# antrea-io/theia

Measured on AMD Instinct MI355X. Metric: flow-records/sec, higher is better.
Workload: dtype u64 (aggregates) + f64 (detectors)

## Files before the change

### theia_amd/csrc/tad_capi.cpp

```cpp
#include "tad_engine.h"

using namespace tad;
using namespace tadh;

namespace tadh {

int ensure_rcp_table(JobCtx *e, uint64_t T) {
  const uint64_t want = T + 2;
  if (want <= e->rcp_n) return TAD_OK;
  uint64_t cap = want < 1024 ? 1024 : want + want / 4;
  int rc = ensure(e, e->rcp_table, cap * sizeof(double));
  if (rc != TAD_OK) return rc;
  std::vector<double> h(cap);
  h[0] = 0.0;
  for (uint64_t i = 1; i < cap; ++i) h[i] = 1.0 / (double)i;
  HIP_TRY(e, hipMemcpyAsync(e->rcp_table.p, h.data(), cap * sizeof(double), hipMemcpyHostToDevice, e->stream));
  HIP_TRY(e, hipStreamSynchronize(e->stream));
  e->rcp_n = cap;
  return TAD_OK;
}

int ensure_key_buffers(JobCtx *e, uint64_t K) {
  int rc;
  const uint64_t k = K ? K : 1;
  if ((rc = ensure(e, e->sigma, k * sizeof(double))) != TAD_OK) return rc;
  if ((rc = ensure(e, e->n_pts, k * sizeof(uint32_t))) != TAD_OK) return rc;
  if ((rc = ensure(e, e->n_anom, k * sizeof(uint32_t))) != TAD_OK) return rc;
  if ((rc = ensure(e, e->off, (k + 1) * sizeof(unsigned long long))) != TAD_OK) return rc;
  if ((rc = ensure(e, e->scan_scratch, scan_scratch_elems(k) * sizeof(unsigned long long))) != TAD_OK) return rc;
  if ((rc = ensure(e, e->key_mean, k * sizeof(double))) != TAD_OK) return rc;
  if ((rc = ensure(e, e->key_m2, k * sizeof(double))) != TAD_OK) return rc;
  if ((rc = ensure(e, e->counters, kTailBytes)) != TAD_OK) return rc;
  return TAD_OK;
}

}

namespace {

template <typename Relaunch>
int arima_yield_loop(JobCtx *e, const unsigned int *yielded_dev, Relaunch relaunch) {
  hipStream_t s = e->stream;
  while (yielded_dev != nullptr && e->eng->pause_dev != nullptr) {
    unsigned int y = 0;
    HIP_TRY(e, hipMemcpyAsync(&y, yielded_dev, 4, hipMemcpyDeviceToHost, s));
    HIP_TRY(e, hipStreamSynchronize(s));
    if (y == 0) break;
    const auto t0 = std::chrono::steady_clock::now();
    while (__atomic_load_n(&e->eng->pause_count, __ATOMIC_ACQUIRE) != 0 && std::chrono::steady_clock::now() - t0 < std::chrono::milliseconds(2))
      std::this_thread::sleep_for(std::chrono::microseconds(50));
    const uint32_t grace = __atomic_load_n(&e->eng->pause_count, __ATOMIC_ACQUIRE) != 0 ? 24u : 0u;
    if (relaunch(grace, &yielded_dev) != 0) return fail(e, TAD_ERR_HIP, "ARIMA launch failed");
    e->arima_relaunches++;
  }
  return TAD_OK;
}

int detect_and_count(JobCtx *e, Grid g, JobParams &jp, DevCounters *ctr, uint64_t *rows, bool stats_done = false) {
  hipStream_t s = e->stream;
  int rc;
  if ((rc = ensure_key_buffers(e, g.K)) != TAD_OK) return rc;
  if ((rc = ensure_rcp_table(e, g.T)) != TAD_OK) return rc;
  double *sigma = static_cast<double *>(e->sigma.p);
  uint32_t *n_pts = static_cast<uint32_t *>(e->n_pts.p);
  uint32_t *n_anom = static_cast<uint32_t *>(e->n_anom.p);
  unsigned long long *off = static_cast<unsigned long long *>(e->off.p);

  const bool ewma = jp.algo == TAD_ALGO_EWMA;
  const bool drop = jp.algo == TAD_ALGO_DROP;
  const bool db_fused = jp.algo == TAD_ALGO_DBSCAN && !jp.all_points && !stats_done && dbscan_uses_list(g);
  jp.lazy_sigma = db_fused;
  if (drop) {
    if ((rc = ensure(e, e->calc, (g.K * g.T ? g.K * g.T : 1) * sizeof(double))) != TAD_OK) return rc;
    launch_drop(s, g, jp.drop_nsigma, jp.drop_min_samples, static_cast<double *>(e->calc.p), sigma, n_pts,
                static_cast<double *>(e->key_mean.p), static_cast<double *>(e->key_m2.p), ctr);
  } else if (!stats_done && !db_fused)
    launch_key_sigma(s, g, jp.alpha, ewma && !jp.all_points, static_cast<const double *>(e->rcp_table.p), sigma, n_pts, n_anom, ctr, static_cast<double *>(e->key_mean.p),
                     static_cast<double *>(e->key_m2.p));
  if (jp.algo == TAD_ALGO_DBSCAN) {
    if ((rc = ensure(e, e->aux, dbscan_scratch_bytes(g))) != TAD_OK) return rc;
    if (dbscan_uses_list(g)) {
      DbscanStats dst{nullptr, nullptr, nullptr, nullptr};
      if (db_fused) dst = DbscanStats{n_pts, n_anom, static_cast<double *>(e->key_mean.p), static_cast<double *>(e->key_m2.p)};
      if (launch_dbscan(s, g, jp.eps, jp.min_samples, e->aux.p, dst, jp.settled && db_fused) != 0)
        return fail(e, TAD_ERR_HIP, "DBSCAN launch failed");
    } else {
      return fail(e, TAD_ERR_GRID_TOO_LARGE, "DBSCAN: series of %llu buckets are not supported", (unsigned long long)g.T);
    }
  } else if (jp.algo == TAD_ALGO_ARIMA) {
    if ((rc = ensure(e, e->calc, g.K * g.T * sizeof(double))) != TAD_OK) return rc;
    const size_t wsb = arima_workspace_bytes(g);
    if ((rc = ensure(e, e->aux, wsb)) != TAD_OK) return rc;
    const bool held = e->hold && e->hold->held;
    if (held) e->hold->release();
    const unsigned int *yielded_dev = nullptr;
    if (launch_arima(s, g, sigma, n_pts, jp.maxiter, static_cast<double *>(e->calc.p), ctr, e->aux.p, wsb, e->eng->pause_dev, &yielded_dev) != 0)
      return fail(e, TAD_ERR_HIP, "ARIMA launch failed");
    if ((rc = arima_yield_loop(e, yielded_dev, [&](uint32_t grace, const unsigned int **yd) {
           return launch_arima_fit(s, g, sigma, n_pts, jp.maxiter, static_cast<double *>(e->calc.p), ctr, e->aux.p, e->eng->pause_dev, yd, grace);
         })) != TAD_OK)
      return rc;
    if (held) e->hold->acquire();
  }
  const uint32_t *cnt = n_anom;
  if (jp.all_points && jp.algo != TAD_ALGO_ARIMA && !drop) cnt = n_pts;
  else if (db_fused) {}
  else if (!ewma || jp.all_points) launch_count_flags(s, g, jp.all_points, n_anom);
  launch_scan_moments(s, cnt, off, g.K, static_cast<unsigned long long *>(e->scan_scratch.p), dev_total(e), n_pts,
                      static_cast<const double *>(e->key_mean.p), static_cast<const double *>(e->key_m2.p), dev_moments(e), db_fused ? ctr : nullptr);
  HIP_TRY(e, hipMemcpyAsync(e->tail_host, e->counters.p, kTailBytes, hipMemcpyDeviceToHost, s));
  HIP_TRY(e, hipStreamSynchronize(s));
  HIP_TRY(e, hipGetLastError());
  *rows = *e->total_host;
  return TAD_OK;
}

}

namespace tadh {

void emit_rows(JobCtx *e, Grid g, Lattice L, const JobParams &jp, OutRows out, uint64_t rows) {
  const int kind = jp.algo == TAD_ALGO_EWMA ? 0 : (jp.algo == TAD_ALGO_ARIMA ? 1 : (jp.algo == TAD_ALGO_DROP ? 3 : (jp.lazy_sigma ? 4 : 2)));
  if (kind == 4 && !jp.all_points &&
      launch_emit_dbscan_list(e->stream, g, L, e->aux.p, static_cast<const uint32_t *>(e->n_anom.p), static_cast<const unsigned long long *>(e->off.p), out))
    return;
  launch_emit(e->stream, g, L, kind, jp.all_points, jp.alpha, static_cast<const double *>(e->sigma.p),
              static_cast<const uint32_t *>(e->n_pts.p), static_cast<const double *>(kind == 3 ? e->key_mean.p : e->calc.p),
              static_cast<const unsigned long long *>(e->off.p), out, rows, e->plan.ewma_emit, e->plan.ewma_emit_rows);
}

}

namespace {

int make_result(JobCtx *e, uint64_t rows, bool with_anomaly, tad_mem out_memory, ResultPriv **out, OutRows *dev_rows,
                ResultBlock *dev_block) {
  ResultPriv *rp = new (std::nothrow) ResultPriv();
  if (!rp) return fail(e, TAD_ERR_OUT_OF_MEMORY, "out of host memory");
  memset(rp, 0, sizeof *rp);
  const size_t bytes = result_bytes(rows, with_anomaly);
  int rc = alloc_device_block(e, bytes, dev_block);
  if (rc != TAD_OK) { delete rp; return rc; }
  carve(dev_block->base, rows, with_anomaly, dev_rows);
  rp->pub.n_rows = rows;
  rp->pub.memory = out_memory;
  *out = rp;
  return TAD_OK;
}

int finish_result(JobCtx *e, ResultPriv *rp, uint64_t rows, bool with_anomaly, ResultBlock dev_block, OutRows dev_rows) {
  if (rp->pub.memory == TAD_MEM_DEVICE) {
    rp->block = dev_block.base;
    rp->block_cap = dev_block.cap;
// ... 265 lines not shown
    const FitListArgs fa{wpos, pcnt, loff, list, hb.nv, pcalc, pflag};
    const bool held = e->hold && e->hold->held;
    if (held) e->hold->release();
    const unsigned int *yielded_dev = nullptr;
    if (launch_arima_stream_fit(s, true, nfits, npos, waves, fpos, ysk, sl, fa, jp.maxiter, ctr, e->as_ws.p, e->eng->pause_dev, &yielded_dev, 0) != 0)
      return fail(e, TAD_ERR_HIP, "ARIMA launch failed");
    if ((rc = arima_yield_loop(e, yielded_dev, [&](uint32_t grace, const unsigned int **yd) {
           return launch_arima_stream_fit(s, false, nfits, npos, waves, fpos, ysk, sl, fa, jp.maxiter, ctr, e->as_ws.p, e->eng->pause_dev, yd, grace);
         })) != TAD_OK)
      return rc;
    if (held) e->hold->acquire();
  }
  launch_as_rows(s, P, hb.nk, tidx, sl.ok, pflag, jp.all_points, rows);
  launch_scan(s, rows, row_off, P, scratch, dev_total(e));
  ab->P = P; ab->tidx = tidx; ab->sigma = sl.sigma; ab->pcalc = pcalc; ab->pflag = pflag; ab->rows = rows; ab->row_off = row_off;
  return TAD_OK;
}

int run_sparse_classes(JobCtx *e, const tad_job *job, const JobParams &jp, bool op_max, uint64_t n_rows_in, uint64_t rows_used, uint64_t K, Lattice L,
                       uint64_t P, uint32_t tmax, tad_mem out_memory, tad_result **out);
int sparse_points_direct(JobCtx *e, uint64_t n_rows_in, uint64_t rows_used, Lattice L, uint64_t P, DevCounters *ctr, tad_mem out_memory,
                         tad_points **points_out);

int run_job(tad_engine *eng, const tad_job *job, const tad_columns *cols, tad_mem out_memory, tad_result **out, tad_points **points_out,
            tad_state *stream = nullptr) {
  tad_engine *e = eng;
  const bool points_mode = points_out != nullptr;
  if (stream && e && job && cols) {
    if (job->algo == TAD_ALGO_DBSCAN && !stream->history)
      return fail(e, TAD_ERR_INVALID_ARGUMENT, "tad_run_stream: DBSCAN needs a state with history (tad_state_create_ex with TAD_STATE_HISTORY)");
    if (job->algo == TAD_ALGO_ARIMA && !stream->series)
      return fail(e, TAD_ERR_INVALID_ARGUMENT, "tad_run_stream: ARIMA needs a state with a series (tad_state_create_ex with TAD_STATE_SERIES)");
    if (job->algo != TAD_ALGO_EWMA && job->algo != TAD_ALGO_DBSCAN && job->algo != TAD_ALGO_ARIMA)
      return fail(e, TAD_ERR_INVALID_ARGUMENT, "tad_run_stream: only the EWMA detector has a streaming form, DBSCAN on a state with history and "
                                               "ARIMA on a state with a series (DROP has none)");
    if (cols->num_keys != stream->K) return fail(e, TAD_ERR_INVALID_ARGUMENT, "tad_run_stream: batch declares %llu keys, the state holds %llu (they must be equal)",
                                                 (unsigned long long)cols->num_keys, (unsigned long long)stream->K);
  }
  if (!e) return fail(nullptr, TAD_ERR_INVALID_ARGUMENT, "tad_run: engine is NULL");
  if (!job || !cols || (!out && !points_out)) return fail(e, TAD_ERR_INVALID_ARGUMENT, "tad_run: job, cols and out must not be NULL");
  if (out) *out = nullptr;
  if (points_out) *points_out = nullptr;
  if (!points_mode && job->algo != TAD_ALGO_EWMA && job->algo != TAD_ALGO_ARIMA && job->algo != TAD_ALGO_DBSCAN && job->algo != TAD_ALGO_DROP)
    return fail(e, TAD_ERR_INVALID_ARGUMENT, "invalid request: Throughput Anomaly Detector algorithm type should be 'EWMA' or 'ARIMA' or 'DBSCAN'");
  if (job->agg_flow < TAD_AGG_NONE || job->agg_flow > TAD_AGG_EXTERNAL)
    return fail(e, TAD_ERR_INVALID_ARGUMENT, "invalid request: Throughput Anomaly Detector aggregated flow type should be 'pod' or 'external' or 'svc'");
  if (job->start_time != 0 && job->end_time != 0 && job->end_time <= job->start_time)
    return fail(e, TAD_ERR_INVALID_ARGUMENT, "invalid request: EndInterval should be after StartInterval");
  if (cols->n_rows > 0 && (!cols->key_id || !cols->flow_end_s || !cols->value))
    return fail(e, TAD_ERR_INVALID_ARGUMENT, "tad_run: key_id, flow_end_s and value columns are required");
  if (cols->n_rows > 0 && cols->num_keys == 0)
    return fail(e, TAD_ERR_INVALID_ARGUMENT, "tad_run: num_keys is 0 but there are rows");
  if ((job->flags & TAD_FLAG_KEY_U32) && cols->num_keys >= 0xFFFFFFFFull)
    return fail(e, TAD_ERR_INVALID_ARGUMENT, "tad_run: TAD_FLAG_KEY_U32 needs num_keys < 2^32 - 1 (TAD_KEY_SKIP32 is the skip marker)");
  if (cols->n_buckets > 0 && cols->step < 1)
    return fail(e, TAD_ERR_INVALID_ARGUMENT, "tad_run: lattice hint needs step >= 1");
  if (job->ewma_alpha < 0.0 || job->ewma_alpha > 1.0 || job->dbscan_eps < 0.0 || job->dbscan_min_samples < 0 || job->arima_maxiter < 0 ||
      job->drop_nsigma < 0.0 || job->drop_min_samples < 0)
    return fail(e, TAD_ERR_INVALID_ARGUMENT, "tad_run: detector parameter out of range");

  std::unique_lock<std::mutex> state_lk;
  if (stream) state_lk = std::unique_lock<std::mutex>(stream->mu);
  if (stream && stream->times_stale)
    return fail(e, TAD_ERR_INVALID_ARGUMENT, "tad_run_stream: the series was imported without its times (tad_state_import_times); state unchanged");
  Lease lease(eng, job->id, !points_mode && job->algo == TAD_ALGO_ARIMA);
  if (!lease.c) return fail(eng, TAD_ERR_OUT_OF_MEMORY, "tad_run: no job context available");
  PauseHold hold(eng);
  lease.c->hold = &hold;
  return run_job_locked(lease.c, job, cols, out_memory, out, points_out, stream, 0);
}

int run_job_locked(JobCtx *e, const tad_job *job, const tad_columns *cols, tad_mem out_memory, tad_result **out, tad_points **points_out,
                   tad_state *stream, int depth) {
  const bool points_mode = points_out != nullptr;
  HIP_TRY(e, hipSetDevice(e->device));
  hipStream_t s = e->stream;
  if (depth == 0) {
    e->done.store(0);
    e->total.store(4);
    e->arima_relaunches = 0;
  }

  JobParams jp;
  jp.algo = job->algo;
  jp.alpha = job->ewma_alpha == 0.0 ? 0.5 : job->ewma_alpha;
  jp.eps = job->dbscan_eps == 0.0 ? 250000000.0 : job->dbscan_eps;
  jp.min_samples = job->dbscan_min_samples == 0 ? 4 : job->dbscan_min_samples;
  jp.maxiter = job->arima_maxiter == 0 ? 50 : job->arima_maxiter;
  jp.drop_nsigma = job->drop_nsigma == 0.0 ? 3.0 : job->drop_nsigma;
  jp.drop_min_samples = job->drop_min_samples == 0 ? 3 : job->drop_min_samples;
  jp.all_points = (job->flags & TAD_FLAG_EMIT_ALL_POINTS) != 0;
  const bool op_max = job->value_op == TAD_OP_MAX || (job->value_op == TAD_OP_AUTO && job->agg_flow == TAD_AGG_NONE);
  const uint64_t n = cols->n_rows;
  const uint64_t K = cols->num_keys;
  RowFilter rf{job->start_time, job->end_time};

  int rc;
  const int cw = ((job->flags & TAD_FLAG_KEY_U32) ? kColKey32 : 0) | ((job->flags & TAD_FLAG_TIME_U32) ? kColTime32 : 0);
  const uint64_t kw = (cw & kColKey32) ? 4 : 8, tw = (cw & kColTime32) ? 4 : 8;
  const void *d_key, *d_key2, *d_te, *d_ts, *d_val;
  if ((rc = stage_column(e, e->in_key, cols->key_id, n, cols->memory, &d_key, kw)) != TAD_OK) return rc;
  if ((rc = stage_column(e, e->in_key2, cols->key_id2, n, cols->memory, &d_key2, kw)) != TAD_OK) return rc;
  if ((rc = stage_column(e, e->in_te, cols->flow_end_s, n, cols->memory, &d_te, tw)) != TAD_OK) return rc;
  if ((rc = stage_column(e, e->in_ts, cols->flow_start_s, n, cols->memory, &d_ts, tw)) != TAD_OK) return rc;
  if ((rc = stage_column(e, e->in_val, cols->value, n, cols->memory, &d_val)) != TAD_OK) return rc;

  if ((rc = ensure(e, e->counters, kTailBytes)) != TAD_OK) return rc;
  DevCounters *ctr = static_cast<DevCounters *>(e->counters.p);

  HIP_TRY(e, hipEventRecord(e->ev[0], s));
  if (depth == 0) HIP_TRY(e, hipEventRecord(e->ev[6], s));
  int lat_mode = cols->n_buckets > 0 ? 0 : 1;
  Lattice L = make_lattice(cols->t0, lat_mode == 0 ? cols->step : 1, cols->n_buckets);
  bool empty = (n == 0 || K == 0);
  const tad_plan plan = e->plan;
  const bool force_v1 = plan.stage0 == 1;
  const bool force_v2 = plan.stage0 == 2;
  const bool has2 = cols->key_id2 != nullptr;
  bool force_v1_retry = false;
  bool force_wide_tiles = plan.tile_cells == 1;
  bool force_exact_hist = plan.histogram == 1;
  bool learnt_exact_hist = false, probing_sampled_hist = false;
  bool kh_rejected = false;
  bool sparse_lsd = plan.sparse_sort == 1;
  {
    const JobCtx::Learnt &lt = e->learnt;
    if (depth == 0 && lt.valid && lt.n == n && lt.K == K && lt.has2 == has2 && lt.algo == (int)job->algo && lt.op == (int)op_max) {
      if (lt.exact_hist) {
        if (lt.exact_uses >= lt.exact_backoff) probing_sampled_hist = true;
        else { force_exact_hist = true; learnt_exact_hist = true; }
      }
      if (lt.wide_tiles) force_wide_tiles = true;
    }
  }
  for (int attempt = 0; attempt < 11; ++attempt) {
    const bool hinted = lat_mode == 0;
    HIP_TRY(e, hipMemsetAsync(ctr, 0, kTailMoments, s));
    jp.settled = false;
    bool narrow_tiles = false;
    PartPlan pl{};
    bool v2 = !empty && !force_v1 && !force_v1_retry && (force_v2 || n >= (1ull << 22)) && part_plan_bins(n, K, has2, &pl);
    if (v2 && e->hold) e->hold->acquire();
    if ((rc = ensure(e, e->meta, sizeof(MetaPartial) * kMetaBlocks)) != TAD_OK) return rc;
    int meta_blocks = 0;
    bool hist_sampled = false;
    const tad_key_hist *kh = cols->key_hist;
    bool use_kh = v2 && depth == 0 && !kh_rejected && kh != nullptr && kh->bins != nullptr && lat_mode != 2 && kh->n_rows == n && kh->num_keys == K &&
                  kh->sides == (has2 ? 2u : 1u) && kh->workgroups == (uint32_t)pl.G && kh->nbins == pl.nbins && kh->shift == (uint32_t)pl.shift_bin &&
                  kh->chunk_rows == pl.chunk && rf.end_time == 0 && !(d_ts != nullptr && rf.start_time != 0);
    const uint32_t *binhist = nullptr;
    if (v2) {
      if ((rc = ensure(e, e->binhist, (size_t)pl.G * pl.nbins * 4)) != TAD_OK) return rc;
      hist_sampled = launch_meta_hist(s, (const uint64_t *)d_key, (const uint64_t *)d_key2, (const int64_t *)d_te, (const int64_t *)d_ts, n, K, rf,
                                      pl, static_cast<MetaPartial *>(e->meta.p), static_cast<uint32_t *>(e->binhist.p), ctr, cw,
                                      use_kh ||
                                      (!force_exact_hist && lat_mode != 2 && sampled_slots_bound(n * (has2 ? 2 : 1), pl) < (1ull << 32) &&
                                          (plan.histogram == 2 ||
                                           n * (has2 ? 2 : 1) / ((uint64_t)pl.G * ((K >> kSampleBlockShift) ? (K >> kSampleBlockShift) : 1)) >= 384)));
      meta_blocks = pl.G;
      binhist = static_cast<const uint32_t *>(e->binhist.p);
      if (use_kh && hist_sampled) { binhist = kh->bins; hist_sampled = false; }
      else use_kh = false;
    }
    if (!hinted && !empty && (!v2 || lat_mode == 2)) {
      meta_blocks = (int)((n + 255) / 256);
      if (meta_blocks > kMetaBlocks) meta_blocks = kMetaBlocks;
      launch_meta(s, (const uint64_t *)d_key, (const uint64_t *)d_key2, (const int64_t *)d_te, (const int64_t *)d_ts, n, rf,
                  static_cast<MetaPartial *>(e->meta.p), meta_blocks, cw);
    }
    if (!hinted && !empty) {
      HIP_TRY(e, hipMemcpyAsync(e->meta_host, e->meta.p, sizeof(MetaPartial) * meta_blocks, hipMemcpyDeviceToHost, s));
      HIP_TRY(e, hipStreamSynchronize(s));
      int64_t tmin = 0, tmax = 0, tref = 0;
      uint64_t g = 0, used = 0;
      for (int b = 0; b < meta_blocks; ++b) {
        const MetaPartial &p = e->meta_host[b];
        if (p.used == 0) continue;
        if (used == 0) { tmin = p.tmin; tmax = p.tmax; tref = p.tref; g = p.g; }
        else {
          if (p.tmin < tmin) tmin = p.tmin;
          if (p.tmax > tmax) tmax = p.tmax;
          const uint64_t d = p.tref >= tref ? (uint64_t)p.tref - (uint64_t)tref : (uint64_t)tref - (uint64_t)p.tref;
          g = host_gcd(host_gcd(g, p.g), d);
        }
        used += p.used;
      }
      if (used == 0 && v2 && lat_mode == 1) {
        lat_mode = 2;
        continue;
      }
      if (used == 0) { empty = true; }
      else {
        const uint64_t span = (uint64_t)tmax - (uint64_t)tmin;
        const uint64_t step = host_gcd(host_gcd(g, span), (uint64_t)tref - (uint64_t)tmin);
        L = make_lattice(tmin, (int64_t)(step == 0 ? 1 : step), span / (step == 0 ? 1 : step) + 1);
      }
    }
    HIP_TRY(e, hipEventRecord(e->ev[1], s));
    if (depth == 0) e->done.store(1);
    if (empty) { L = make_lattice(0, 1, 0); v2 = false; }

    uint64_t cells = empty ? 0 : K * L.nb;
    const bool cells_overflow = !empty && L.nb != 0 && cells / L.nb != K;
    uint64_t need = cells * 9 + (jp.algo == TAD_ALGO_ARIMA ? cells * 80 + (1ull << 22) : (jp.algo == TAD_ALGO_DROP ? cells * 8 : 0));
    const uint64_t slots_all = n * (has2 ? 2 : 1);
    bool sparse = !empty && K <= 0xFFFFFFFFull && slots_all < (1ull << 32) &&
                  (plan.sparse == 2 ||
                   (plan.sparse != 1 && (cells_overflow || need > e->ws_limit || (cells >= (1ull << 24) && slots_all < cells / 8))));
    Grid sparse_grid{};
    bool sp_part = false;
    const unsigned long long *stream_poff = nullptr;
    uint64_t stream_P = 0;
    if (sparse && use_kh) {
      kh_rejected = true;
      continue;
    }
    if (sparse) {
      PartPlan spl = pl;
      sp_part = v2 && !sparse_lsd && part_plan_sparse(K, L.nb, has2, &spl);
      if (sp_part) {
        part_plan_wc(slots_all, columns_aligned16(d_key, d_key2, d_te, d_val), has2, 2, &spl);
        if (spl.wc_cap == 0 || slots_all + spl.pad_slots >= (1ull << 32)) sp_part = false;
      }
      if (sp_part && hist_sampled) { force_exact_hist = true; continue; }
      v2 = false;
      const uint64_t stage_slots = slots_all + (sp_part ? spl.pad_slots : 0);
      if ((rc = ensure(e, e->sp_comp_a, stage_slots * 8)) != TAD_OK) return rc;
      if ((rc = ensure(e, e->sp_comp_b, stage_slots * 8)) != TAD_OK) return rc;
      if ((rc = ensure(e, e->sp_val_a, stage_slots * 8)) != TAD_OK) return rc;
      if ((rc = ensure(e, e->sp_val_b, stage_slots * 8)) != TAD_OK) return rc;
      size_t tb = sparse_sort_temp_bytes(slots_all);
      if (sp_part && sparse_part_temp_bytes(spl) > tb) tb = sparse_part_temp_bytes(spl);
      if ((uint64_t)slots_all * 32 + tb > e->ws_limit)
        return fail(e, TAD_ERR_GRID_TOO_LARGE, "sparse Stage 0 needs %llu bytes of sort buffers for %llu row slots > workspace limit %llu",
                    (unsigned long long)(slots_all * 32 + tb), (unsigned long long)slots_all, (unsigned long long)e->ws_limit);
      if ((rc = ensure(e, e->sp_temp, tb + 64)) != TAD_OK) return rc;
      if ((rc = ensure(e, e->sp_first, K * 4 + 64)) != TAD_OK) return rc;
      unsigned long long *d_runs = reinterpret_cast<unsigned long long *>(static_cast<unsigned char *>(e->sp_temp.p) + tb);
      HIP_TRY(e, hipMemsetAsync(d_runs, 0, 16, s));
      HIP_TRY(e, hipEventRecord(e->ev[2], s));
      unsigned long long *ucomp = static_cast<unsigned long long *>(e->sp_comp_a.p), *uval = static_cast<unsigned long long *>(e->sp_val_a.p);
      const uint64_t span = L.nb ? (L.nb - 1) * (uint64_t)L.step : 0;
      if (sp_part) {
        const uint64_t slots = slots_all + spl.pad_slots;
        if ((rc = ensure(e, e->part_total, (size_t)spl.nparts * 4)) != TAD_OK) return rc;
        if ((rc = ensure(e, e->part_start, ((size_t)spl.nparts + 1) * 8)) != TAD_OK) return rc;
        if ((rc = ensure(e, e->part_offs32, (size_t)spl.G * spl.nparts * 4)) != TAD_OK) return rc;
        if ((rc = ensure(e, e->recs, (size_t)slots * 8)) != TAD_OK) return rc;
        if ((rc = ensure(e, e->slices, slice_table_bytes(slots, spl))) != TAD_OK) return rc;
        uint32_t *offs32 = static_cast<uint32_t *>(e->part_offs32.p);
        unsigned long long *part_start = static_cast<unsigned long long *>(e->part_start.p);
        launch_part_offsets(s, binhist, spl, offs32, static_cast<uint32_t *>(e->part_total.p), part_start, false,
                            static_cast<const MetaPartial *>(e->meta.p), n, slots, e->slices.p, Grid{});
        launch_partition(s, (const uint64_t *)d_key, (const uint64_t *)d_key2, (const int64_t *)d_te, (const int64_t *)d_ts, (const uint64_t *)d_val, n, K,
                         rf, L, spl, offs32, part_start, e->recs.p, nullptr, dev_ovf_count(e), 0, ctr, nullptr, nullptr, cw);
        launch_sparse_sort(s, e->recs.p, part_start, binhist, spl, K, L.step, op_max,
                           ucomp, static_cast<unsigned long long *>(e->sp_comp_b.p), static_cast<unsigned long long *>(e->sp_val_b.p),
                           reinterpret_cast<uint32_t *>(uval), e->sp_temp.p, d_runs, ctr);
      } else if (launch_sparse_group(s, (const uint64_t *)d_key, (const uint64_t *)d_key2, (const int64_t *)d_te, (const int64_t *)d_ts, (const uint64_t *)d_val, n, K,
                                     rf, L.t0, span, op_max, ucomp, uval, static_cast<unsigned long long *>(e->sp_comp_b.p),
                                     static_cast<unsigned long long *>(e->sp_val_b.p), e->sp_temp.p, tb, d_runs, ctr, cw) != 0)
        return fail(e, TAD_ERR_HIP, "sparse Stage 0: sort / reduce failed");
      if (depth == 0) e->sp_by_partition = sp_part;
      if (!sp_part) launch_sparse_tmax(s, ucomp, slots_all, d_runs, static_cast<uint32_t *>(e->sp_first.p), reinterpret_cast<unsigned int *>(d_runs + 1));
      unsigned long long runs_tmax[2] = {0, 0};
      HIP_TRY(e, hipMemcpyAsync(runs_tmax, d_runs, 16, hipMemcpyDeviceToHost, s));
      if (sp_part) HIP_TRY(e, hipMemcpyAsync(e->ctr_host, ctr, sizeof(DevCounters), hipMemcpyDeviceToHost, s));
      HIP_TRY(e, hipStreamSynchronize(s));
      if (sp_part) {
        const uint32_t er = e->ctr_host->err;
        if (er & DEV_ERR_KEY_RANGE)
          return fail(e, TAD_ERR_KEY_RANGE, "a key id is >= num_keys (%llu) and is not TAD_KEY_SKIP", (unsigned long long)K);
        if (er & DEV_ERR_OFF_LATTICE) {
          if (lat_mode < 2) { lat_mode = (lat_mode == 0) ? 1 : 2; continue; }
          return fail(e, TAD_ERR_HIP, "internal error: a row fell off the derived time lattice");
        }
        if (er & (DEV_ERR_OVERFLOW_LIST | DEV_ERR_SPARSE_ROUND)) { sparse_lsd = true; continue; }
      }
      const uint64_t P = runs_tmax[0];
      const unsigned int tmax = (unsigned int)runs_tmax[1];
      if (stream) {
        if (sp_part) {
          launch_sparse_compact(s, spl, e->sp_temp.p, static_cast<const unsigned long long *>(e->sp_comp_b.p), static_cast<const unsigned long long *>(e->sp_val_b.p), ucomp, uval);
          launch_sparse_tmax(s, ucomp, slots_all, d_runs, static_cast<uint32_t *>(e->sp_first.p), reinterpret_cast<unsigned int *>(d_runs + 1));
        }
        if ((rc = ensure_key_buffers(e, K)) != TAD_OK) return rc;
        const size_t kpad = (size_t)((K + 3) & ~3ull);
        if ((rc = ensure(e, e->sp_cls, kpad * 4 + (K + 1) * 8 + 64)) != TAD_OK) return rc;
        uint32_t *len = static_cast<uint32_t *>(e->sp_cls.p);
        unsigned long long *poff = reinterpret_cast<unsigned long long *>(len + kpad);
        HIP_TRY(e, hipMemsetAsync(len, 0, (size_t)K * 4, s));
        launch_sparse_len(s, ucomp, P, static_cast<const uint32_t *>(e->sp_first.p), len);
        launch_scan(s, len, poff, K, static_cast<unsigned long long *>(e->scan_scratch.p), nullptr);
        stream_poff = poff;
        stream_P = P;
        sparse_grid = Grid{nullptr, nullptr, K, 0, nullptr};
        HIP_TRY(e, hipEventRecord(e->ev[3], s));
      } else {
        cells = K * (uint64_t)tmax;
        need = cells * 17 + (jp.algo == TAD_ALGO_ARIMA ? cells * 80 + (1ull << 22) : (jp.algo == TAD_ALGO_DROP ? cells * 8 : 0));
        if (P && depth == 0 && (need > e->ws_limit || plan.sparse_classes == 1)) {
          if (sp_part) {
            launch_sparse_compact(s, spl, e->sp_temp.p, static_cast<const unsigned long long *>(e->sp_comp_b.p), static_cast<const unsigned long long *>(e->sp_val_b.p), ucomp, uval);
            launch_sparse_tmax(s, ucomp, slots_all, d_runs, static_cast<uint32_t *>(e->sp_first.p), reinterpret_cast<unsigned int *>(d_runs + 1));
          }
          HIP_TRY(e, hipMemcpyAsync(e->ctr_host, ctr, sizeof(DevCounters), hipMemcpyDeviceToHost, s));
          HIP_TRY(e, hipStreamSynchronize(s));
          const DevCounters c0 = *e->ctr_host;
          if (c0.err & DEV_ERR_KEY_RANGE)
            return fail(e, TAD_ERR_KEY_RANGE, "a key id is >= num_keys (%llu) and is not TAD_KEY_SKIP", (unsigned long long)K);
          if (c0.err & DEV_ERR_OFF_LATTICE) {
            if (lat_mode < 2) { lat_mode = (lat_mode == 0) ? 1 : 2; continue; }
            return fail(e, TAD_ERR_HIP, "internal error: a row fell off the derived time lattice");
          }
          if (points_mode) return sparse_points_direct(e, n, c0.rows_used, L, P, ctr, out_memory, points_out);
          return run_sparse_classes(e, job, jp, op_max, n, c0.rows_used, K, L, P, tmax, out_memory, out);
        }
        if (need > e->ws_limit)
          return fail(e, TAD_ERR_GRID_TOO_LARGE, "sparse point grid needs %llu bytes (%llu keys x longest series %u points) > workspace limit %llu",
                      (unsigned long long)need, (unsigned long long)K, tmax, (unsigned long long)e->ws_limit);
        if ((rc = ensure(e, e->grid_val, (cells ? cells : 1) * 8)) != TAD_OK) return rc;
        if ((rc = ensure(e, e->grid_flag, cells ? cells : 1)) != TAD_OK) return rc;
        if ((rc = ensure(e, e->sp_times, (cells ? cells : 1) * 8)) != TAD_OK) return rc;
        sparse_grid = Grid{static_cast<unsigned long long *>(e->grid_val.p), static_cast<uint8_t *>(e->grid_flag.p), tmax ? K : 0, tmax,
// ... 1034 lines not shown
```

### theia_amd/csrc/tad_stage0_part.hip

```cpp
#include <cstdlib>
#include <cstring>

#include "tad_internal.h"

namespace tad {

static constexpr int kPartThreads = 1024;

static constexpr int kMinCellBits = 15, kMaxCellBits = 24;
static constexpr uint32_t kTileCells = 17744;
static constexpr uint32_t kMaxParts = 2048;
static constexpr size_t kLdsBudget = 156 * 1024;
static constexpr int kGcdSamples = 4;

__device__ __forceinline__ void lds_barrier() { asm volatile("s_waitcnt lgkmcnt(0)\n\ts_barrier" ::: "memory"); }

__device__ __forceinline__ uint64_t p_gcd_u64(uint64_t a, uint64_t b) {
  if (a == 0) return b;
  if (b == 0) return a;
  if (((a | b) >> 32) == 0) {
    uint32_t x = (uint32_t)a, y = (uint32_t)b;
    while (y) { uint32_t r = x % y; x = y; y = r; }
    return x;
  }
  while (b) { uint64_t r = a % b; a = b; b = r; }
  return a;
}

__device__ __forceinline__ uint64_t p_absdiff(int64_t a, int64_t b) {
  return a >= b ? (uint64_t)a - (uint64_t)b : (uint64_t)b - (uint64_t)a;
}

struct PMeta {
  int64_t tmin, tmax, tref;
  uint64_t g, used;
};

__device__ __forceinline__ PMeta pmeta_merge(PMeta a, const PMeta &b) {
  if (b.used == 0) return a;
  if (a.used == 0) return b;
  a.tmin = b.tmin < a.tmin ? b.tmin : a.tmin;
  a.tmax = b.tmax > a.tmax ? b.tmax : a.tmax;
  a.g = p_gcd_u64(p_gcd_u64(a.g, b.g), p_absdiff(a.tref, b.tref));
  a.used += b.used;
  return a;
}

__device__ __forceinline__ bool p_time_kept(int64_t te, int64_t ts, bool has_ts, RowFilter f) {
  if (f.end_time != 0 && !(te < f.end_time)) return false;
  if (f.start_time != 0 && has_ts && !(ts >= f.start_time)) return false;
  return true;
}

__device__ __forceinline__ bool p_bucket(const Lattice &L, int64_t te, uint32_t &bucket) {
  const uint64_t d = (uint64_t)te - (uint64_t)L.t0;
  uint64_t b;
  if (L.mode == 0) b = d;
  else if (L.mode == 1) { if (d >> 32) return false; b = __umul64hi(d, L.magic); }
  else b = d / (uint64_t)L.step;
  if (b >= L.nb || b * (uint64_t)L.step != d) return false;
  bucket = (uint32_t)b;
  return true;
}

struct MetaAcc {
  PMeta m;
  int nsample;
  uint32_t err;
};

#ifndef TAD_WAVE_AGG
#define TAD_WAVE_AGG 1
#endif
#ifndef TAD_ADAPTIVE_QUEUES
#define TAD_ADAPTIVE_QUEUES 1
#endif
#ifndef TAD_WAVE_AGG_MIN
#define TAD_WAVE_AGG_MIN 8
#endif
static constexpr int kWaveAggMin = TAD_WAVE_AGG_MIN;
static constexpr size_t kWcFixedBytes = 18;

__device__ __forceinline__ void hist_add(uint32_t *hist, uint32_t bin, uint32_t weight) {
#if TAD_WAVE_AGG
  const uint32_t b0 = __builtin_amdgcn_readfirstlane(bin);
  const unsigned long long grp = __ballot(bin == b0);
  if (__popcll(grp) >= kWaveAggMin && bin == b0) {
    if (__builtin_amdgcn_mbcnt_hi((uint32_t)(grp >> 32), __builtin_amdgcn_mbcnt_lo((uint32_t)grp, 0u)) == 0) atomicAdd(&hist[b0], (uint32_t)__popcll(grp) * weight);
    return;
  }
#endif
  atomicAdd(&hist[bin], weight);
}

__device__ __forceinline__ void meta_row(MetaAcc &a, uint32_t *hist, uint64_t k1, uint64_t k2, int64_t te, bool kept,
                                         uint64_t K, int shift_bin, uint32_t weight = 1u) {
  if (!kept) return;
  bool counted = false;
  if (k1 != TAD_KEY_SKIP) {
    if (k1 < K) { hist_add(hist, (uint32_t)(k1 >> shift_bin), weight); counted = true; }
    else a.err |= DEV_ERR_KEY_RANGE;
  }
  if (k2 != TAD_KEY_SKIP) {
    if (k2 < K) { hist_add(hist, (uint32_t)(k2 >> shift_bin), weight); counted = true; }
    else a.err |= DEV_ERR_KEY_RANGE;
  }
  if (!counted) return;
  if (a.m.used == 0) {
    a.m.tmin = a.m.tmax = a.m.tref = te;
    a.m.g = 0;
  } else {
    a.m.tmin = te < a.m.tmin ? te : a.m.tmin;
    a.m.tmax = te > a.m.tmax ? te : a.m.tmax;
    if (a.nsample < kGcdSamples) {
      const uint64_t d = p_absdiff(te, a.m.tref);
      if (d != 0) { a.m.g = p_gcd_u64(a.m.g, d); a.nsample++; }
    }
  }
  a.m.used++;
}

__device__ __forceinline__ void hist_row(MetaAcc &a, uint32_t *hist, uint64_t k1, uint64_t k2, uint64_t K, int shift_bin) {
  if (k1 != TAD_KEY_SKIP) {
    if (k1 < K) hist_add(hist, (uint32_t)(k1 >> shift_bin), 1u);
    else a.err |= DEV_ERR_KEY_RANGE;
  }
  if (k2 != TAD_KEY_SKIP) {
    if (k2 < K) hist_add(hist, (uint32_t)(k2 >> shift_bin), 1u);
    else a.err |= DEV_ERR_KEY_RANGE;
  }
}

#ifndef TAD_SAMPLE_MASK
#define TAD_SAMPLE_MASK 15
#endif
#ifndef TAD_REGION_UR
#define TAD_REGION_UR 12
#endif
static constexpr uint32_t kSampleMask = TAD_SAMPLE_MASK;

template <bool VEC, bool HAS2, bool SAMPLE_H, bool K32 = false, bool T32 = false>
__global__ __launch_bounds__(kPartThreads) void k_meta_hist(const uint64_t *__restrict__ key,
                                                            const uint64_t *__restrict__ key2,
                                                            const int64_t *__restrict__ t_end,
                                                            const int64_t *__restrict__ t_start,
                                                            uint64_t n, uint64_t chunk, uint64_t K, RowFilter f,
                                                            int shift_bin, uint32_t nbins,
                                                            MetaPartial *__restrict__ partials,
                                                            uint32_t *__restrict__ binhist, DevCounters *ctr) {
  extern __shared__ __attribute__((aligned(16))) unsigned char smem[];
  uint32_t *hist = reinterpret_cast<uint32_t *>(smem);
  for (uint32_t i = threadIdx.x; i < nbins; i += kPartThreads) hist[i] = 0;
  __syncthreads();
  const uint64_t lo = (uint64_t)blockIdx.x * chunk;
  const uint64_t hi = lo + chunk < n ? lo + chunk : n;
  MetaAcc acc{{0, 0, 0, 0, 0}, 0, 0};
  uint32_t seen = 0;
  const bool has_ts = t_start != nullptr && f.start_time != 0;
  if (VEC) {
    const uint64_t npair = hi > lo ? (hi - lo) >> 1 : 0;
    const ulonglong2 *kv = reinterpret_cast<const ulonglong2 *>(key + lo);
    const ulonglong2 *k2v = reinterpret_cast<const ulonglong2 *>(key2 + (HAS2 ? lo : 0));
    const longlong2 *tv = reinterpret_cast<const longlong2 *>(t_end + lo);
    auto kpair = [&](const ulonglong2 *wide, const uint64_t *col, uint64_t j) -> ulonglong2 {
      if constexpr (K32) return ld_key2<true>(col, lo, j);
      else return wide[j];
    };
    auto tpair = [&](uint64_t j) -> longlong2 {
      if constexpr (T32) return ld_time2<true>(t_end, lo, j);
      else return tv[j];
    };
    constexpr int U = 4;
    const bool sample_t = SAMPLE_H || (f.end_time == 0 && !has_ts);
    uint64_t i = threadIdx.x;
    uint32_t it = 0;
    for (; i + (U - 1) * kPartThreads < npair; i += U * kPartThreads, ++it) {
      const bool zone = (i - threadIdx.x) + 2 * U * kPartThreads >= npair;
      const bool with_t = !sample_t || zone || (it & kSampleMask) == ((threadIdx.x >> 6) & kSampleMask);
      if (SAMPLE_H && !with_t) continue;
      const uint32_t weight = SAMPLE_H && !zone ? kSampleMask + 1u : 1u;
      seen += 2 * U;
      ulonglong2 k[U], k2[U];
      longlong2 t[U];
#pragma unroll
      for (int u = 0; u < U; ++u) {
        k[u] = kpair(kv, key, i + u * kPartThreads);
        k2[u] = HAS2 ? kpair(k2v, key2, i + u * kPartThreads) : make_ulonglong2(TAD_KEY_SKIP, TAD_KEY_SKIP);
      }
      if (with_t) {
#pragma unroll
        for (int u = 0; u < U; ++u) t[u] = tpair(i + u * kPartThreads);
#pragma unroll
        for (int u = 0; u < U; ++u) {
          const uint64_t r = lo + 2 * (i + u * kPartThreads);
          const int64_t ts0 = has_ts ? ld_time<T32>(t_start, r) : 0, ts1 = has_ts ? ld_time<T32>(t_start, r + 1) : 0;
          meta_row(acc, hist, k[u].x, k2[u].x, t[u].x, p_time_kept(t[u].x, ts0, has_ts, f), K, shift_bin, weight);
          meta_row(acc, hist, k[u].y, k2[u].y, t[u].y, p_time_kept(t[u].y, ts1, has_ts, f), K, shift_bin, weight);
        }
      } else {
#pragma unroll
        for (int u = 0; u < U; ++u) {
          hist_row(acc, hist, k[u].x, k2[u].x, K, shift_bin);
          hist_row(acc, hist, k[u].y, k2[u].y, K, shift_bin);
        }
      }
    }
    for (; i < npair; i += kPartThreads) {
      seen += 2;
      const ulonglong2 k = kpair(kv, key, i);
      const longlong2 t = tpair(i);
      const ulonglong2 k2 = HAS2 ? kpair(k2v, key2, i) : make_ulonglong2(TAD_KEY_SKIP, TAD_KEY_SKIP);
      const uint64_t r = lo + 2 * i;
      const int64_t ts0 = has_ts ? ld_time<T32>(t_start, r) : 0, ts1 = has_ts ? ld_time<T32>(t_start, r + 1) : 0;
      meta_row(acc, hist, k.x, k2.x, t.x, p_time_kept(t.x, ts0, has_ts, f), K, shift_bin);
      meta_row(acc, hist, k.y, k2.y, t.y, p_time_kept(t.y, ts1, has_ts, f), K, shift_bin);
    }
    if (((hi - lo) & 1) && threadIdx.x == 0 && hi > lo) {
      seen += 1;
      const uint64_t r = hi - 1;
      const int64_t te = ld_time<T32>(t_end, r);
      meta_row(acc, hist, ld_key<K32>(key, r), HAS2 ? ld_key<K32>(key2, r) : TAD_KEY_SKIP, te, p_time_kept(te, has_ts ? ld_time<T32>(t_start, r) : 0, has_ts, f), K, shift_bin);
    }
  } else {
    for (uint64_t r = lo + threadIdx.x; r < hi; r += kPartThreads) {
      seen += 1;
      const int64_t te = ld_time<T32>(t_end, r);
      meta_row(acc, hist, ld_key<K32>(key, r), HAS2 ? ld_key<K32>(key2, r) : TAD_KEY_SKIP, te, p_time_kept(te, has_ts ? ld_time<T32>(t_start, r) : 0, has_ts, f), K, shift_bin);
    }
  }
  PMeta m = acc.m;
  uint32_t err = acc.err;
  unsigned long long seen_w = seen;
  for (int d = 32; d >= 1; d >>= 1) seen_w += __shfl_down(seen_w, d);
  for (int d = 32; d >= 1; d >>= 1) {
    PMeta o;
    o.tmin = __shfl_down((long long)m.tmin, d);
    o.tmax = __shfl_down((long long)m.tmax, d);
    o.tref = __shfl_down((long long)m.tref, d);
    o.g = __shfl_down((unsigned long long)m.g, d);
    o.used = __shfl_down((unsigned long long)m.used, d);
    m = pmeta_merge(m, o);
    err |= __shfl_down(err, d);
  }
  __shared__ PMeta s_acc[kPartThreads / 64];
  __shared__ uint32_t s_err[kPartThreads / 64];
  __shared__ unsigned long long s_seen[kPartThreads / 64];
  const int lane = threadIdx.x & 63, wave = threadIdx.x >> 6;
  if (lane == 0) { s_acc[wave] = m; s_err[wave] = err; s_seen[wave] = seen_w; }
  __syncthreads();
  if (threadIdx.x == 0) {
    PMeta a = s_acc[0];
    uint32_t e = s_err[0];
    unsigned long long sn = s_seen[0];
    for (int w = 1; w < kPartThreads / 64; ++w) { a = pmeta_merge(a, s_acc[w]); e |= s_err[w]; sn += s_seen[w]; }
    MetaPartial p;
    p.tmin = a.tmin; p.tmax = a.tmax; p.tref = a.tref; p.g = a.g; p.used = a.used; p.seen = sn;
    partials[blockIdx.x] = p;
    if (e) atomicOr(&ctr->err, e);
  }
  uint32_t *out = binhist + (size_t)blockIdx.x * nbins;
  for (uint32_t i = threadIdx.x; i < nbins; i += kPartThreads) out[i] = hist[i];
}

static constexpr double kCapSigmas = 5.5, kCapIntervals = 12.0;
__device__ __forceinline__ uint32_t sampled_capacity(uint32_t est) {
  constexpr double scale = (double)(kSampleMask + 1);
  return (uint32_t)((double)est + kCapSigmas * sqrt((double)est * scale) + kCapIntervals * scale);
}
static constexpr uint32_t kBigSampledRegion = 8192;

struct SliceTable {
  uint32_t *slice_part;
  uint32_t *slice_first;
  uint32_t *n_slices;
};

struct OffsetsArgs {
  const uint32_t *binhist;
  uint32_t nbins, bins_per_part, nparts, round_mask;
  int G;
  const MetaPartial *partials;
  uint64_t n, chunk;
  uint32_t *offs32;
  uint32_t *total;
  unsigned long long *part_start;
  SliceTable st;
  uint32_t slice_len;
  Grid g;
  int shift_part;
  DevCounters *ctr;
};

__global__ __launch_bounds__(256) void k_part_offsets(OffsetsArgs A) {
  const uint32_t lane = threadIdx.x & 63u, wave = threadIdx.x >> 6;
  const uint32_t p = blockIdx.x * 4u + wave;
  const uint32_t per = (uint32_t)(A.G + 63) / 64u;
  if (p < A.nparts) {
    const uint32_t b0 = p * A.bins_per_part;
    const uint32_t b1 = b0 + A.bins_per_part < A.nbins ? b0 + A.bins_per_part : A.nbins;
    auto count_of = [&](uint32_t gi) -> uint32_t {
      const uint32_t *row = A.binhist + (size_t)gi * A.nbins;
      uint32_t c = 0;
      for (uint32_t b = b0; b < b1; ++b) c += row[b];
      if (A.partials != nullptr) c = sampled_capacity(c);
      return (c + A.round_mask) & ~A.round_mask;
    };
    constexpr uint32_t kKeep = 4;
    uint32_t kept[kKeep] = {0, 0, 0, 0};
    uint32_t sum = 0;
    if (per <= kKeep) {
#pragma unroll
      for (uint32_t j = 0; j < kKeep; ++j) {
        const uint32_t gi = lane * per + j;
        if (j < per && gi < (uint32_t)A.G) { kept[j] = count_of(gi); sum += kept[j]; }
      }
    } else {
      for (uint32_t j = 0; j < per; ++j) {
        const uint32_t gi = lane * per + j;
        if (gi < (uint32_t)A.G) sum += count_of(gi);
      }
    }
    uint32_t incl = sum;
    for (int d = 1; d < 64; d <<= 1) { const uint32_t y = __shfl_up(incl, d); if (lane >= (uint32_t)d) incl += y; }
    uint32_t run = incl - sum;
    const uint32_t tot = __shfl(incl, 63);
    if (per <= kKeep) {
#pragma unroll
      for (uint32_t j = 0; j < kKeep; ++j) {
        const uint32_t gi = lane * per + j;
        if (j < per && gi < (uint32_t)A.G) { A.offs32[(size_t)gi * A.nparts + p] = run; run += kept[j]; }
      }
    } else {
      for (uint32_t j = 0; j < per; ++j) {
        const uint32_t gi = lane * per + j;
        if (gi < (uint32_t)A.G) { A.offs32[(size_t)gi * A.nparts + p] = run; run += count_of(gi); }
      }
    }
    if (lane == 0) A.total[p] = tot;
    if (A.partials != nullptr && A.ctr != nullptr) {
      bool big = false;
      if (per <= kKeep) {
#pragma unroll
        for (uint32_t j = 0; j < kKeep; ++j) big |= kept[j] > kBigSampledRegion && (unsigned long long)kept[j] * (unsigned)A.G > 8ull * tot;
      } else {
        for (uint32_t j = 0; j < per; ++j) {
          const uint32_t gi = lane * per + j;
          if (gi < (uint32_t)A.G) { const uint32_t c = count_of(gi); big |= c > kBigSampledRegion && (unsigned long long)c * (unsigned)A.G > 8ull * tot; }
        }
      }
      if (__any(big) && lane == 0) atomicOr(&A.ctr->err, DEV_ERR_REGION_FULL);
    }
    if (tot > A.slice_len) {
      const uint32_t KP = 1u << A.shift_part;
      const uint64_t k0 = (uint64_t)p << A.shift_part, cells_all = (uint64_t)KP * A.g.T;
      for (uint64_t c = lane; c < cells_all; c += 64) {
        const uint64_t b = c >> A.shift_part, k = k0 + (c & (KP - 1));
        if (k < A.g.K) { A.g.val[b * A.g.K + k] = 0ull; A.g.flag[b * A.g.K + k] = 0; }
      }
    }
  }
}

__global__ __launch_bounds__(256) void k_part_tail(OffsetsArgs A) {
  const uint32_t lane = threadIdx.x & 63u, wave = threadIdx.x >> 6;
  __shared__ uint32_t s_wave[4];
  const uint32_t F = A.nparts;
  constexpr uint32_t kEach = 8;
  const uint32_t f0 = threadIdx.x * kEach;
  uint32_t tot[kEach];
#pragma unroll
  for (uint32_t j = 0; j < kEach; ++j) tot[j] = f0 + j < F ? A.total[f0 + j] : 0u;
  auto nsl = [&](uint32_t t) -> uint32_t { const uint32_t k = (uint32_t)(((unsigned long long)t + A.slice_len - 1) / A.slice_len); return k ? k : 1u; };
  unsigned long long rsum = 0;
  uint32_t ssum = 0;
#pragma unroll
  for (uint32_t j = 0; j < kEach; ++j)
    if (f0 + j < F) { rsum += tot[j]; ssum += nsl(tot[j]); }
  unsigned long long rincl = rsum;
  uint32_t sincl = ssum;
  for (int d = 1; d < 64; d <<= 1) {
    const unsigned long long y = __shfl_up(rincl, d);
    const uint32_t z = __shfl_up(sincl, d);
    if (lane >= (uint32_t)d) { rincl += y; sincl += z; }
  }
  __shared__ unsigned long long s_r[4];
  if (lane == 63) { s_r[wave] = rincl; s_wave[wave] = sincl; }
  __syncthreads();
  unsigned long long rbase = 0, rtot = 0;
  uint32_t sbase = 0, stot = 0;
  for (uint32_t w = 0; w < 4; ++w) {
    if (w < wave) { rbase += s_r[w]; sbase += s_wave[w]; }
    rtot += s_r[w]; stot += s_wave[w];
  }
  unsigned long long rrun = rbase + rincl - rsum;
  uint32_t srun = sbase + sincl - ssum;
#pragma unroll
  for (uint32_t j = 0; j < kEach; ++j) {
    const uint32_t q = f0 + j;
    if (q < F) {
      A.part_start[q] = rrun;
      rrun += tot[j];
      const uint32_t k = nsl(tot[j]);
      A.st.slice_first[q] = srun;
      for (uint32_t i = 0; i < k; ++i) A.st.slice_part[srun + i] = q;
      srun += k;
    }
  }
  if (threadIdx.x == 0) { A.part_start[F] = rtot; *A.st.n_slices = (A.ctr != nullptr && (A.ctr->err & DEV_ERR_REGION_FULL)) ? 0u : stot; }
}

__device__ __forceinline__ void block_count_rows(uint32_t used, uint32_t err, DevCounters *ctr) {
  __shared__ unsigned long long s_u[kPartThreads / 64];
  __shared__ uint32_t s_e[kPartThreads / 64];
  unsigned long long u = used;
  for (int d = 32; d >= 1; d >>= 1) { u += __shfl_down(u, d); err |= __shfl_down(err, d); }
  if ((threadIdx.x & 63) == 0) { s_u[threadIdx.x >> 6] = u; s_e[threadIdx.x >> 6] = err; }
  __syncthreads();
  if (threadIdx.x == 0) {
    for (int w = 1; w < kPartThreads / 64; ++w) { u += s_u[w]; err |= s_e[w]; }
    if (u) atomicAdd(&ctr->rows_used, u);
    if (err) atomicOr(&ctr->err, err);
  }
}

struct PartArgs {
  const uint64_t *key, *key2;
  const int64_t *t_end, *t_start;
  const uint64_t *value;
  uint64_t n, chunk, K;
  RowFilter f;
  Lattice L;
  int shift_part;
  uint32_t kp_mask;
  int cell_bits;
  uint32_t nparts;
  const uint32_t *offs32;
  const unsigned long long *part_start;
  unsigned long long *recs;
  OverflowRec *ovf;
  unsigned long long *ovf_count;
  uint32_t ovf_cap;
  DevCounters *ctr;
  uint32_t *fin;
  int G;
  unsigned long long value_limit;
  unsigned long long narrow_limit;
  uint32_t *ovf_keys;
};

__device__ __forceinline__ void lds_exclusive_scan(uint32_t *a, uint32_t n, uint32_t *s_wave) {
  const uint32_t per = (n + kPartThreads - 1) / kPartThreads;
  const uint32_t b0 = threadIdx.x * per;
  uint32_t sum = 0;
  for (uint32_t j = 0; j < per; ++j)
    if (b0 + j < n) sum += a[b0 + j];
  const int lane = threadIdx.x & 63, wave = threadIdx.x >> 6;
// ... 1079 lines not shown
```

Baseline: 77.87 billion.

## Write meta partials directly to host memory, tree-merge waves, vectorize offsets

The meta-histogram kernel now writes per-block partials straight into the host-visible meta buffer, which drops the device-to-host copy before the stream sync. The block-level merge of per-wave partials now runs as a shuffle tree in wave 0 instead of a serial loop in thread 0. The partition-offsets kernel sums bin-histogram rows with 128-bit vector loads when alignment allows. Debug knockout switches are also added but default off. Risk: writing to host memory from the kernel depends on meta_host being device-accessible pinned memory, and each of those writes crosses PCIe.

```diff
diff --git a/theia_amd/csrc/tad_capi.cpp b/theia_amd/csrc/tad_capi.cpp
--- a/theia_amd/csrc/tad_capi.cpp
+++ b/theia_amd/csrc/tad_capi.cpp
@@ -1,4 +1,8 @@
 #include "tad_engine.h"
+
+#ifndef TAD_META_DIRECT
+#define TAD_META_DIRECT 1
+#endif
 
 using namespace tad;
 using namespace tadh;
@@ -570,7 +574,7 @@
     if (v2) {
       if ((rc = ensure(e, e->binhist, (size_t)pl.G * pl.nbins * 4)) != TAD_OK) return rc;
       hist_sampled = launch_meta_hist(s, (const uint64_t *)d_key, (const uint64_t *)d_key2, (const int64_t *)d_te, (const int64_t *)d_ts, n, K, rf,
-                                      pl, static_cast<MetaPartial *>(e->meta.p), static_cast<uint32_t *>(e->binhist.p), ctr, cw,
+                                      pl, TAD_META_DIRECT ? e->meta_host : static_cast<MetaPartial *>(e->meta.p), static_cast<uint32_t *>(e->binhist.p), ctr, cw,
                                       use_kh ||
                                       (!force_exact_hist && lat_mode != 2 && sampled_slots_bound(n * (has2 ? 2 : 1), pl) < (1ull << 32) &&
                                           (plan.histogram == 2 ||
@@ -587,7 +591,8 @@
                   static_cast<MetaPartial *>(e->meta.p), meta_blocks, cw);
     }
     if (!hinted && !empty) {
-      HIP_TRY(e, hipMemcpyAsync(e->meta_host, e->meta.p, sizeof(MetaPartial) * meta_blocks, hipMemcpyDeviceToHost, s));
+      if (!(TAD_META_DIRECT && v2 && lat_mode != 2))
+        HIP_TRY(e, hipMemcpyAsync(e->meta_host, e->meta.p, sizeof(MetaPartial) * meta_blocks, hipMemcpyDeviceToHost, s));
       HIP_TRY(e, hipStreamSynchronize(s));
       int64_t tmin = 0, tmax = 0, tref = 0;
       uint64_t g = 0, used = 0;
diff --git a/theia_amd/csrc/tad_stage0_part.hip b/theia_amd/csrc/tad_stage0_part.hip
--- a/theia_amd/csrc/tad_stage0_part.hip
+++ b/theia_amd/csrc/tad_stage0_part.hip
@@ -93,16 +93,28 @@
   atomicAdd(&hist[bin], weight);
 }
 
+#ifndef TAD_PASS_A_KNOCKOUT
+#define TAD_PASS_A_KNOCKOUT 0
+#endif
+#ifndef TAD_OFFSETS_VEC4
+#define TAD_OFFSETS_VEC4 1
+#endif
+#ifndef TAD_PASS_A_TREE_MERGE
+#define TAD_PASS_A_TREE_MERGE 1
+#endif
+
+template <int KO = 0>
 __device__ __forceinline__ void meta_row(MetaAcc &a, uint32_t *hist, uint64_t k1, uint64_t k2, int64_t te, bool kept,
                                          uint64_t K, int shift_bin, uint32_t weight = 1u) {
+  if (KO & 16) { a.m.tref ^= (int64_t)(k1 ^ k2) ^ te; return; }
   if (!kept) return;
   bool counted = false;
   if (k1 != TAD_KEY_SKIP) {
-    if (k1 < K) { hist_add(hist, (uint32_t)(k1 >> shift_bin), weight); counted = true; }
+    if (k1 < K) { if (!(KO & 8)) hist_add(hist, (uint32_t)(k1 >> shift_bin), weight); counted = true; }
     else a.err |= DEV_ERR_KEY_RANGE;
   }
   if (k2 != TAD_KEY_SKIP) {
-    if (k2 < K) { hist_add(hist, (uint32_t)(k2 >> shift_bin), weight); counted = true; }
+    if (k2 < K) { if (!(KO & 8)) hist_add(hist, (uint32_t)(k2 >> shift_bin), weight); counted = true; }
     else a.err |= DEV_ERR_KEY_RANGE;
   }
   if (!counted) return;
@@ -112,7 +124,7 @@
   } else {
     a.m.tmin = te < a.m.tmin ? te : a.m.tmin;
     a.m.tmax = te > a.m.tmax ? te : a.m.tmax;
-    if (a.nsample < kGcdSamples) {
+    if (!(KO & 4) && a.nsample < kGcdSamples) {
       const uint64_t d = p_absdiff(te, a.m.tref);
       if (d != 0) { a.m.g = p_gcd_u64(a.m.g, d); a.nsample++; }
     }
@@ -154,6 +166,7 @@
   __syncthreads();
   const uint64_t lo = (uint64_t)blockIdx.x * chunk;
   const uint64_t hi = lo + chunk < n ? lo + chunk : n;
+  constexpr int KO = SAMPLE_H ? TAD_PASS_A_KNOCKOUT : 0;
   MetaAcc acc{{0, 0, 0, 0, 0}, 0, 0};
   uint32_t seen = 0;
   const bool has_ts = t_start != nullptr && f.start_time != 0;
@@ -178,6 +191,7 @@
       const bool zone = (i - threadIdx.x) + 2 * U * kPartThreads >= npair;
       const bool with_t = !sample_t || zone || (it & kSampleMask) == ((threadIdx.x >> 6) & kSampleMask);
       if (SAMPLE_H && !with_t) continue;
+      if ((KO & 1) && zone) continue;
       const uint32_t weight = SAMPLE_H && !zone ? kSampleMask + 1u : 1u;
       seen += 2 * U;
       ulonglong2 k[U], k2[U];
@@ -194,8 +208,8 @@
         for (int u = 0; u < U; ++u) {
           const uint64_t r = lo + 2 * (i + u * kPartThreads);
           const int64_t ts0 = has_ts ? ld_time<T32>(t_start, r) : 0, ts1 = has_ts ? ld_time<T32>(t_start, r + 1) : 0;
-          meta_row(acc, hist, k[u].x, k2[u].x, t[u].x, p_time_kept(t[u].x, ts0, has_ts, f), K, shift_bin, weight);
-          meta_row(acc, hist, k[u].y, k2[u].y, t[u].y, p_time_kept(t[u].y, ts1, has_ts, f), K, shift_bin, weight);
+          meta_row<KO>(acc, hist, k[u].x, k2[u].x, t[u].x, p_time_kept(t[u].x, ts0, has_ts, f), K, shift_bin, weight);
+          meta_row<KO>(acc, hist, k[u].y, k2[u].y, t[u].y, p_time_kept(t[u].y, ts1, has_ts, f), K, shift_bin, weight);
         }
       } else {
 #pragma unroll
@@ -205,27 +219,27 @@
         }
       }
     }
-    for (; i < npair; i += kPartThreads) {
+    for (; !(KO & 2) && i < npair; i += kPartThreads) {
       seen += 2;
       const ulonglong2 k = kpair(kv, key, i);
       const longlong2 t = tpair(i);
       const ulonglong2 k2 = HAS2 ? kpair(k2v, key2, i) : make_ulonglong2(TAD_KEY_SKIP, TAD_KEY_SKIP);
       const uint64_t r = lo + 2 * i;
       const int64_t ts0 = has_ts ? ld_time<T32>(t_start, r) : 0, ts1 = has_ts ? ld_time<T32>(t_start, r + 1) : 0;
-      meta_row(acc, hist, k.x, k2.x, t.x, p_time_kept(t.x, ts0, has_ts, f), K, shift_bin);
-      meta_row(acc, hist, k.y, k2.y, t.y, p_time_kept(t.y, ts1, has_ts, f), K, shift_bin);
+      meta_row<KO>(acc, hist, k.x, k2.x, t.x, p_time_kept(t.x, ts0, has_ts, f), K, shift_bin);
+      meta_row<KO>(acc, hist, k.y, k2.y, t.y, p_time_kept(t.y, ts1, has_ts, f), K, shift_bin);
     }
     if (((hi - lo) & 1) && threadIdx.x == 0 && hi > lo) {
       seen += 1;
       const uint64_t r = hi - 1;
       const int64_t te = ld_time<T32>(t_end, r);
-      meta_row(acc, hist, ld_key<K32>(key, r), HAS2 ? ld_key<K32>(key2, r) : TAD_KEY_SKIP, te, p_time_kept(te, has_ts ? ld_time<T32>(t_start, r) : 0, has_ts, f), K, shift_bin);
+      meta_row<KO>(acc, hist, ld_key<K32>(key, r), HAS2 ? ld_key<K32>(key2, r) : TAD_KEY_SKIP, te, p_time_kept(te, has_ts ? ld_time<T32>(t_start, r) : 0, has_ts, f), K, shift_bin);
     }
   } else {
     for (uint64_t r = lo + threadIdx.x; r < hi; r += kPartThreads) {
       seen += 1;
       const int64_t te = ld_time<T32>(t_end, r);
-      meta_row(acc, hist, ld_key<K32>(key, r), HAS2 ? ld_key<K32>(key2, r) : TAD_KEY_SKIP, te, p_time_kept(te, has_ts ? ld_time<T32>(t_start, r) : 0, has_ts, f), K, shift_bin);
+      meta_row<KO>(acc, hist, ld_key<K32>(key, r), HAS2 ? ld_key<K32>(key2, r) : TAD_KEY_SKIP, te, p_time_kept(te, has_ts ? ld_time<T32>(t_start, r) : 0, has_ts, f), K, shift_bin);
     }
   }
   PMeta m = acc.m;
@@ -248,16 +262,44 @@
   const int lane = threadIdx.x & 63, wave = threadIdx.x >> 6;
   if (lane == 0) { s_acc[wave] = m; s_err[wave] = err; s_seen[wave] = seen_w; }
   __syncthreads();
+#if TAD_PASS_A_TREE_MERGE
+  if (wave == 0) {
+    constexpr int kWaves = kPartThreads / 64;
+    const int src = lane < kWaves ? lane : 0;
+    PMeta a = s_acc[src];
+    uint32_t e = s_err[src];
+    unsigned long long sn = s_seen[src];
+    if (lane >= kWaves || ((KO & 32) && lane != 0)) { a.used = 0; e = 0; sn = 0; }
+    for (int d = kWaves / 2; d >= 1; d >>= 1) {
+      PMeta o;
+      o.tmin = __shfl_down((long long)a.tmin, d);
+      o.tmax = __shfl_down((long long)a.tmax, d);
+      o.tref = __shfl_down((long long)a.tref, d);
+      o.g = __shfl_down((unsigned long long)a.g, d);
+      o.used = __shfl_down((unsigned long long)a.used, d);
+      a = pmeta_merge(a, o);
+      e |= __shfl_down(e, d);
+      sn += __shfl_down(sn, d);
+    }
+    if (lane == 0) {
+      MetaPartial p;
+      p.tmin = a.tmin; p.tmax = a.tmax; p.tref = a.tref; p.g = a.g; p.used = a.used; p.seen = sn;
+      partials[blockIdx.x] = p;
+      if (e) atomicOr(&ctr->err, e);
+    }
+  }
+#else
   if (threadIdx.x == 0) {
     PMeta a = s_acc[0];
     uint32_t e = s_err[0];
     unsigned long long sn = s_seen[0];
-    for (int w = 1; w < kPartThreads / 64; ++w) { a = pmeta_merge(a, s_acc[w]); e |= s_err[w]; sn += s_seen[w]; }
+    for (int w = 1; w < ((KO & 32) ? 1 : kPartThreads / 64); ++w) { a = pmeta_merge(a, s_acc[w]); e |= s_err[w]; sn += s_seen[w]; }
     MetaPartial p;
     p.tmin = a.tmin; p.tmax = a.tmax; p.tref = a.tref; p.g = a.g; p.used = a.used; p.seen = sn;
     partials[blockIdx.x] = p;
     if (e) atomicOr(&ctr->err, e);
   }
+#endif
   uint32_t *out = binhist + (size_t)blockIdx.x * nbins;
   for (uint32_t i = threadIdx.x; i < nbins; i += kPartThreads) out[i] = hist[i];
 }
@@ -298,10 +340,15 @@
   if (p < A.nparts) {
     const uint32_t b0 = p * A.bins_per_part;
     const uint32_t b1 = b0 + A.bins_per_part < A.nbins ? b0 + A.bins_per_part : A.nbins;
+    const bool vec4 = TAD_OFFSETS_VEC4 && ((A.nbins | A.bins_per_part) & 3u) == 0 && (reinterpret_cast<uintptr_t>(A.binhist) & 15) == 0;
     auto count_of = [&](uint32_t gi) -> uint32_t {
       const uint32_t *row = A.binhist + (size_t)gi * A.nbins;
       uint32_t c = 0;
-      for (uint32_t b = b0; b < b1; ++b) c += row[b];
+      if (vec4) {
+        for (uint32_t b = b0; b < b1; b += 4) { const uint4 v = *reinterpret_cast<const uint4 *>(row + b); c += v.x + v.y + v.z + v.w; }
+      } else {
+        for (uint32_t b = b0; b < b1; ++b) c += row[b];
+      }
       if (A.partials != nullptr) c = sampled_capacity(c);
       return (c + A.round_mask) & ~A.round_mask;
     };
```

After: 78.32 billion, median of 6. No clear change (+0.6%).
